# Anttwo/MACARONS

Measured on AMD Instinct MI355X. Metric: candidate-camera coverage-gain evals/sec (100k pts, 200 cams), higher is better.
Workload: dtype f32; 1 GPU; scorer: B=1 cloud x N=100000 points x C=200 cameras per GPU (BASELINE headline 100k pts / 200 cams), inputs resident in HBM; points=100000, cams_per_gpu=200, parallelism=camera-shard x1, streams=2

## Files before the change

### macarons_amd/csrc/networks.hip

```cpp
#include "nn_kernels.h"
#include "net_layout.h"
#include <cstdlib>
#include <algorithm>
#include <map>
#include <mutex>
#include <utility>

namespace mcr {

#ifdef MCR_DEV_LOCAL_PCT8
void launch_local_pct8(hipStream_t s, const float* offs, float* feat, int64_t ld_feat, int64_t S, const float* blob);
#define MCR_VARIANT8_OK(v) ((v) == 8)
#else
#define MCR_VARIANT8_OK(v) false
#endif
static int g_default_variant = []() {
    const char* e = getenv("MCR_LOCAL_PCT_VARIANT");
    const int v = e ? atoi(e) : 6;
    return (v == 1 || v == 5 || v == 6) ? v : 6;
}();
static thread_local int t_next_variant = 0;
static thread_local int t_variant = 0;
static thread_local int t_scope_depth = 0;
struct VariantScope {
// ... 474 lines not shown
        launch_linear3p(s, fP, W2, {fc2.b, ACT_GELU}, h128, T, 128, VIS_E, np);
        launch_linear3p(s, h128, W3, {fc3.b, ACT_NONE}, {out, 64}, T, 64, 128, np);
    } else {
        launch_layernorm(s, x, VIS_E, w.ng, w.nb, h, VIS_E, T, VIS_E);
        launch_linear(s, {h, VIS_E}, {fc1.w, VIS_E}, {fc1.b, ACT_GELU}, {ff, VIS_E}, T, 192, VIS_E, seq_route(N));
        launch_copy2d(s, view_harmonics, 64, ff + 192, VIS_E, T, 64);
        launch_linear(s, {ff, VIS_E}, {fc2.w, VIS_E}, {fc2.b, ACT_GELU}, {h, 128}, T, 128, VIS_E, seq_route(N));
        launch_linear(s, {h, 128}, {fc3.w, 128}, {fc3.b, ACT_NONE}, {out, 64}, T, 64, 128, N);
    }
    MCR_LAUNCH_CHECK("mcr_scone_vis_forward");
    return 0;
}

constexpr int OCC_CHUNK = 16384;
constexpr int FEAT = 1344;
constexpr size_t OCC_WS_SLACK = 8192 + 2 * 1024, OCC_RAGGED_WS_SLACK = 8192 + 1024;

struct OccHead {
    float *feat, *h1, *h2, *gfeat, *gbias;
    void* wplanes;
    HeadScratch planes() const { return HeadScratch{reinterpret_cast<_Float16*>(feat), reinterpret_cast<_Float16*>(h1), h2, wplanes}; }
};
static OccHead carve_occ_head(Arena& a, int64_t T, int64_t G) {
    OccHead w;
    w.feat = a.f(T * FEAT);
    w.h1 = a.f(T * 512);
    w.h2 = a.f(T * 256);
    w.gfeat = a.f(G * 512);
    w.gbias = a.f(G * 512);
    w.wplanes = a.bytes(linear3h_planes_bytes(512, 1344));
    return w;
}

struct OccSide { hipStream_t s = nullptr; hipEvent_t fork = nullptr, join = nullptr; };
static OccSide* occ_side(hipStream_t caller, int slot = 0) {
    static const bool on = []() { const char* e = getenv("MCR_OCC_OVERLAP"); return !(e && e[0] == '0'); }();
    if (!on) return nullptr;
    static std::mutex mu;
    static std::map<std::pair<std::pair<int, int>, hipStream_t>, OccSide> table;
    int dev = 0;
    if (hipGetDevice(&dev) != hipSuccess) return nullptr;
    std::lock_guard<std::mutex> lock(mu);
    OccSide& x = table[std::make_pair(std::make_pair(dev, slot), caller)];
    if (!x.s) {
        if (hipStreamCreateWithFlags(&x.s, hipStreamNonBlocking) != hipSuccess || hipEventCreateWithFlags(&x.fork, hipEventDisableTiming) != hipSuccess ||
            hipEventCreateWithFlags(&x.join, hipEventDisableTiming) != hipSuccess) {
            x.s = nullptr;
            return nullptr;
        }
    }
    return &x;
}
static hipStream_t fork_side(hipStream_t s, OccSide*& side) {
    if (side && hipEventRecord(side->fork, s) == hipSuccess && hipStreamWaitEvent(side->s, side->fork, 0) == hipSuccess) return side->s;
    side = nullptr;
    return s;
}
struct SideJoin {
    OccSide* side; hipStream_t s; bool recorded = false, joined = false;
    ~SideJoin() {
        if (!side || joined) return;
        if (!recorded) (void)hipEventRecord(side->join, side->s);
        (void)hipStreamWaitEvent(s, side->join, 0);
    }
};

static void run_global(hipStream_t gs, const OccW& w, const float* pc_global, int64_t G, int64_t Lg, const int* lens, const EncScratch& glob,
                       const OccHead& hd) {
    run_pct(gs, w.global, pc_global, hd.gfeat, 512, G, (int)Lg, 256, glob, lens);
    launch_linear(gs, {hd.gfeat, 512}, {w.lin1.w, 1856}, {nullptr, ACT_NONE}, {hd.gbias, 512}, G, 512, 512, 1);
}

static void head_linear(hipStream_t s, int which, Rows X, const LinW& lin, int64_t ldw, RowsOut Y, int64_t M, int N, int K, RowBias rb,
                        const void* const* head_planes, const float* head_inv_scales, void* wplanes) {
    const int variant = g_local_pct_variant;
    const int64_t ANY_M = (int64_t)1 << 40;
    const Rows W{lin.w, ldw};
    const Epilogue e{lin.b, ACT_GELU, {}, rb};
    if ((variant == 6 || variant == 7) && linear3h_applicable(X.p, X.ld, W.p, W.ld, ANY_M, N, K))
        launch_linear3h(s, X, head_weight_planes(s, which, lin, ldw, N, K, head_planes, head_inv_scales, wplanes), e, Y, M, N, K);
    else if (variant == 5 && linear3_applicable(X.p, X.ld, W.p, W.ld, ANY_M, N, K))
        launch_linear3(s, X, W, e, Y, M, N, K);
    else
        launch_linear(s, X, W, e, Y, M, N, K, 1);
}

static int run_occ_head(const char* who, hipStream_t s, const OccW& w, const float* x, const float* view_harmonics, int64_t T, const OccHead& hd,
                        int64_t rows_per_group, const int* row_group, const void* const* head_planes, const float* head_inv_scales, bool planes,
                        bool x_done, OccSide* side, SideJoin& side_join, int* range_flag, float* out) {
    bool join_failed = false;
    auto join = [&]() {
        if (side) {
            side_join.joined = true;
            join_failed = hipStreamWaitEvent(s, side->join, 0) != hipSuccess;
        }
    };
    if (planes)
        run_head_planes(s, x, view_harmonics, T, w.xe1, w.xe2, w.xe3, w.lin1, w.lin2, w.lin3, hd.gbias, rows_per_group, row_group, head_planes,
                        head_inv_scales, hd.planes(), out, join, x_done);
    else {
        launch_linear(s, {x, 3}, {w.xe1.w, 3}, {w.xe1.b, ACT_GELU}, {hd.h2, 128}, T, 128, 3, 1);
        head_linear(s, 0, {hd.h2, 128}, w.xe2, 128, {hd.h1, 256}, T, 256, 128, {}, head_planes, head_inv_scales, hd.wplanes);
        head_linear(s, 1, {hd.h1, 256}, w.xe3, 256, {hd.feat + 768, FEAT}, T, 512, 256, {}, head_planes, head_inv_scales, hd.wplanes);
        launch_copy2d(s, view_harmonics, 64, hd.feat + 1280, FEAT, T, 64);
        join();
        MCR_REQUIRE(!join_failed, "%s: side stream (join)", who);
        head_linear(s, 2, {hd.feat, FEAT}, {w.lin1.w + 512, w.lin1.b}, 1856, {hd.h1, 512}, T, 512, FEAT, {hd.gbias, rows_per_group, row_group},
                    head_planes, head_inv_scales, hd.wplanes);
        head_linear(s, 3, {hd.h1, 512}, w.lin2, 512, {hd.h2, 256}, T, 256, 512, {}, head_planes, head_inv_scales, hd.wplanes);
        launch_linear(s, {hd.h2, 256}, {w.lin3.w, 256}, {w.lin3.b, ACT_GELU}, {out, 1}, T, 1, 256, 1);
    }
    MCR_REQUIRE(!join_failed, "%s: side stream (join)", who);
    if (range_flag) launch_nonfinite_flag(s, out, T, range_flag);
    MCR_LAUNCH_CHECK(who);
    return 0;
}

struct OccLocal { float* offs; EncScratch pct; };
static OccLocal carve_occ_local(Arena& a, int64_t rows, bool layer_by_layer) {
    OccLocal w{};
    w.offs = a.f(rows * 16 * 3);
    if (layer_by_layer) w.pct = carve_enc(a, rows * 16, PCT_E);
    return w;
}
struct OccScratch {
    OccHead head;
    char *knn_q, *knn_c, *knn_park;
    size_t knn_c_bytes;
    EncScratch glob;
    Arena scratch;
};
static OccScratch carve_occ(Arena& a, int64_t B, int64_t Q, int64_t Lg) {
    OccScratch w;
    w.head = carve_occ_head(a, B * Q, B);
    w.knn_c_bytes = knn_grid_cloud_bytes(B, 16384);
    w.knn_q = (char*)a.bytes(knn_grid_query_bytes(B, Q));
    w.knn_c = (char*)a.bytes(3 * w.knn_c_bytes);
    w.knn_park = (char*)a.bytes(knn_grid_park_bytes());
    w.glob = carve_enc(a, B * Lg, PCT_E);
    w.scratch = a.rest();
    return w;
}
size_t mcr_scone_occ_workspace_bytes(int64_t B, int64_t Q, int64_t Lg) {
    const size_t local = std::max({measure(carve_occ_local, B * Q, false), measure(carve_occ_local, Q, false),
                                   measure(carve_occ_local, std::min<int64_t>(Q, OCC_CHUNK), true)});
    return measure(carve_occ, B, Q, Lg) + local + OCC_WS_SLACK;
}

int mcr_knn_points(const float* X, const float* pc, int64_t* idx, float* dists, float* pts, int64_t B, int64_t Q, int64_t M,
                   int k, int subtract_query, void* stream);

int mcr_scone_occ_forward_phase(const float* pc_global, int64_t Lg, const float* const* pc_scale, const int64_t* M_scale,
                                const float* x, const float* view_harmonics, float* out, int64_t B, int64_t Q,
                                const float* const* weights, int n_weights, const float* const* local_blobs,
                                const void* const* head_planes, const float* head_inv_scales, int* range_flag, void* workspace,
                                size_t workspace_bytes, int phase, void* stream) {
    const char* who = "mcr_scone_occ_forward";
    VariantScope variant_scope_;
    MCR_REQUIRE(phase >= 0 && phase <= 2, "mcr_scone_occ_forward: phase must be 0, 1 or 2");
    const bool early = phase != 2, late = phase != 1;
    MCR_REQUIRE(pc_scale && M_scale && x && weights && (!late || (pc_global && view_harmonics && out)), "mcr_scone_occ_forward: null pointer");
    MCR_REQUIRE(!head_planes || head_inv_scales, "mcr_scone_occ_forward: head_planes need head_inv_scales");
    if (check_table(who, OCC_TABLE, weights, n_weights, n_weights)) return 1;
    MCR_REQUIRE(B > 0 && Q > 0 && Lg > 0 && B <= 65535, "mcr_scone_occ_forward: bad problem size");
    MCR_REQUIRE(workspace && workspace_bytes >= mcr_scone_occ_workspace_bytes(B, Q, Lg), "mcr_scone_occ_forward: workspace too small");
    for (int i = 0; i < 3; ++i)
        MCR_REQUIRE((pc_scale[i] || (!late && i > 0)) && M_scale[i] >= 16, "mcr_scone_occ_forward: scale %d has %ld points (< k = 16)", i,
                    (long)M_scale[i]);
    hipStream_t s = (hipStream_t)stream;
    const OccW w = read_occ_table(weights, n_weights);
    Arena arena{(char*)workspace, workspace_bytes};
    const OccScratch ws = carve_occ(arena, B, Q, Lg);
    MCR_REQUIRE(arena.ok(), "mcr_scone_occ_forward: workspace overflow (global)");
    const OccHead& hd = ws.head;
    float* feat = hd.feat;

    OccSide* side = late ? occ_side(s) : nullptr;
    const hipStream_t gs = fork_side(s, side);
    SideJoin side_join{side, s};
    const bool fused_all = local_blobs && local_blobs[0] && local_blobs[1] && local_blobs[2];
    const int64_t qc = fused_all ? Q : std::min<int64_t>(Q, OCC_CHUNK);
    const bool planes = fused_all && fp16_planes_variant();
    const int64_t Tall = B * Q;
    const Planes featP = planes_over(hd.feat, Tall, FEAT);
    OccSide* xside = planes ? occ_side(s, 1) : nullptr;
    struct XJoin {
        OccSide* side; hipStream_t s; bool armed;
        bool wait() { if (!armed) return true; armed = false; return hipStreamWaitEvent(s, side->join, 0) == hipSuccess; }
        ~XJoin() { (void)wait(); }
    } x_join{xside, s, false};
    if (xside && early) {
        MCR_REQUIRE(hipEventRecord(xside->fork, s) == hipSuccess && hipStreamWaitEvent(xside->s, xside->fork, 0) == hipSuccess,
                    "mcr_scone_occ_forward: side stream (x embedding fork)");
        run_x_embedding_planes(xside->s, x, nullptr, B * Q, w.xe1, w.xe2, w.xe3, head_planes, head_inv_scales, hd.planes());
        MCR_REQUIRE(hipEventRecord(xside->join, xside->s) == hipSuccess, "mcr_scone_occ_forward: side stream (x embedding record)");
        x_join.armed = true;
    }
    if (late) {
        run_global(gs, w, pc_global, B, Lg, nullptr, ws.glob, hd);
        if (xside)
            launch_split_to_planes(gs, {view_harmonics, 64}, featP.cols(1280).keep(matrix_planes()), B * Q, 64);
    }
    if (side) {
        MCR_REQUIRE(hipEventRecord(side->join, side->s) == hipSuccess, "mcr_scone_occ_forward: side stream (record)");
        side_join.recorded = true;
    }
    const int* knn_qperm = nullptr;
    KnnGridCloud knn_clouds[3]{};
    int knn_slot[3] = {-1, -1, -1};
    if (qc == Q) {
        const float* g_pc[3]; int64_t g_M[3]; void* g_ws[3];
        int n_grid = 0;
        for (int sc = 0; sc < 3; ++sc)
            if (knn_grid_applicable(M_scale[sc], 16)) {
                g_pc[n_grid] = pc_scale[sc]; g_M[n_grid] = M_scale[sc]; g_ws[n_grid] = ws.knn_c + n_grid * ws.knn_c_bytes;
                knn_slot[sc] = n_grid++;
            }
        if (n_grid) {
            if (phase == 0) {
                knn_qperm = knn_grid_order_queries(s, x, B, Q, ws.knn_q, ws.knn_park);
                knn_grid_build_clouds(s, n_grid, g_pc, g_M, B, g_ws, knn_clouds);
            } else {
                const int first = early ? 0 : (knn_slot[0] >= 0 ? 1 : 0), count = early ? (knn_slot[0] >= 0 ? 1 : 0) : n_grid - first;
                OccSide* bside = early && count > 0 ? occ_side(s) : nullptr;
                const hipStream_t bs = fork_side(s, bside);
                knn_grid_build_clouds(bs, count, g_pc + first, g_M + first, B, g_ws + first, knn_clouds + first);
                const bool recorded = !bside || hipEventRecord(bside->join, bside->s) == hipSuccess;
                knn_qperm = knn_grid_order_queries(s, x, B, Q, ws.knn_q, ws.knn_park, early);
                const bool joined = !bside || hipStreamWaitEvent(s, bside->join, 0) == hipSuccess;
                MCR_REQUIRE(recorded && joined, "mcr_scone_occ_forward: side stream (cloud build)");
            }
            MCR_LAUNCH_CHECK("knn grid preparation");
        }
    }
    for (int sc = 0; sc < 3; ++sc) {
        if (sc == 0 ? !early : !late) continue;
        const bool grid_knn = knn_slot[sc] >= 0;
        const KnnGridCloud knn_cloud = grid_knn ? knn_clouds[knn_slot[sc]] : KnnGridCloud{};
        const bool fused = planes || (local_blobs && local_blobs[sc]);
        if (B > 1 && qc == Q && fused) {
            Arena a = ws.scratch;
            float* offs = carve_occ_local(a, Tall, false).offs;
            MCR_REQUIRE(a.ok(), "mcr_scone_occ_forward: workspace overflow (kNN)");
            if (grid_knn) {
                launch_knn16_grid(s, x, pc_scale[sc], M_scale[sc], knn_qperm, knn_cloud, 0, B, Q, nullptr, nullptr, offs, true, ws.knn_park, sc);
                MCR_LAUNCH_CHECK("knn_grid_kernel");
            } else if (int e = mcr_knn_points(x, pc_scale[sc], nullptr, nullptr, offs, B, Q, M_scale[sc], 16, 1, stream))
                return e;
            if (planes) run_local_pct(s, offs, nullptr, FEAT, Tall, local_blobs[sc], featP.cols(sc * 256));
            else run_local_pct(s, offs, feat + sc * 256, FEAT, Tall, local_blobs[sc]);
            continue;
        }
        for (int64_t q0 = 0; q0 < Q; q0 += qc) {
            const int64_t nq = std::min<int64_t>(qc, Q - q0);
            for (int64_t b = 0; b < B; ++b) {
                Arena a = ws.scratch;
                const OccLocal loc = carve_occ_local(a, nq, !fused);
                MCR_REQUIRE(a.ok(), fused ? "mcr_scone_occ_forward: workspace overflow (kNN)" : "mcr_scone_occ_forward: workspace overflow (local)");
                float* offs = loc.offs;
                if (grid_knn) {
                    launch_knn16_grid(s, x, pc_scale[sc], M_scale[sc], knn_qperm, knn_cloud, b, 1, Q, nullptr, nullptr, offs, true, ws.knn_park,
                                      (int)(sc * B + b));
                    MCR_LAUNCH_CHECK("knn_grid_kernel");
                } else if (int e = mcr_knn_points(x + (b * Q + q0) * 3, pc_scale[sc] + b * M_scale[sc] * 3, nullptr, nullptr, offs, 1, nq,
                                                  M_scale[sc], 16, 1, stream))
                    return e;
                if (planes)
                    run_local_pct(s, offs, nullptr, FEAT, nq, local_blobs[sc], featP.cols((b * Q + q0) * FEAT + sc * 256));
                else if (fused)
                    run_local_pct(s, offs, feat + (b * Q + q0) * FEAT + sc * 256, FEAT, nq, local_blobs[sc]);
                else
                    run_pct(s, w.local[sc], offs, feat + (b * Q + q0) * FEAT + sc * 256, FEAT, nq, 16, 128, loc.pct);
            }
        }
    }
    MCR_REQUIRE(x_join.wait(), "mcr_scone_occ_forward: side stream (x embedding join)");
    if (!late) {
        MCR_LAUNCH_CHECK("mcr_scone_occ_forward (phase 1)");
        return 0;
    }
    return run_occ_head(who, s, w, x, view_harmonics, Tall, hd, Q, nullptr, head_planes, head_inv_scales, planes, xside != nullptr, side,
                        side_join, range_flag, out);
}

int mcr_scone_occ_forward(const float* pc_global, int64_t Lg, const float* const* pc_scale, const int64_t* M_scale,
                          const float* x, const float* view_harmonics, float* out, int64_t B, int64_t Q,
                          const float* const* weights, int n_weights, const float* const* local_blobs,
                          const void* const* head_planes, const float* head_inv_scales, int* range_flag, void* workspace,
                          size_t workspace_bytes, void* stream) {
    return mcr_scone_occ_forward_phase(pc_global, Lg, pc_scale, M_scale, x, view_harmonics, out, B, Q, weights, n_weights, local_blobs,
                                       head_planes, head_inv_scales, range_flag, workspace, workspace_bytes, 0, stream);
}

struct OccRaggedScratch { OccHead head; EncScratch glob; float *offs, *knn_split; };
static OccRaggedScratch carve_occ_ragged(Arena& a, int64_t J, int64_t T, int64_t Lg) {
    OccRaggedScratch w;
    w.head = carve_occ_head(a, T, J);
    w.glob = carve_enc(a, J * Lg, PCT_E);
    w.offs = a.f(T * 16 * 3);
    w.knn_split = a.f(knn16_segmented_split_floats(T));
    return w;
}
size_t mcr_scone_occ_ragged_workspace_bytes(int64_t J, int64_t T, int64_t Lg) { return measure(carve_occ_ragged, J, T, Lg) + OCC_RAGGED_WS_SLACK; }
int mcr_knn_rows_per_block(void) { return knn_rows_per_block(); }

int mcr_scone_occ_forward_ragged_phase(const float* pc_global, const int* global_len, int64_t Lg, const float* const* pc_scale,
                                       const int64_t* const* scale_off, const float* x, const float* view_harmonics, const int* row_job,
                                       const int* knn_blocks, int64_t n_blocks, float* out, int64_t J, int64_t T,
                                       const float* const* weights, int n_weights, const float* const* local_blobs,
                                       const void* const* head_planes, const float* head_inv_scales, int* range_flag, void* workspace,
                                       size_t workspace_bytes, int phase, void* stream) {
// ... 61 lines not shown
```

### macarons_amd/nbv.py

```python

import torch

from . import dist as mdist
from .utility import scone_utils as su


class ViewStateGrid:

    def __init__(self, device, degree=8, n_elev=7, n_azim=14):
        self.n_elev, self.n_azim = n_elev, n_azim
        self.base_harmonics, self.h_polar, self.h_azim = su.get_all_harmonics_under_degree(degree, n_elev, n_azim, device)


_side_streams = {}


def _harmonics_beside(scone_occ, pc, Xl, harmonics_of):
    dev = Xl.device
    main = torch.cuda.current_stream(dev)
    fork = torch.cuda.Event()
    fork.record(main)
    begun = scone_occ.forward_begin(pc, Xl)
    if begun is None:
        return begun, harmonics_of(Xl)
    side = _side_streams.get((dev.index, main.cuda_stream))
    if side is None:
        side = _side_streams[(dev.index, main.cuda_stream)] = torch.cuda.Stream(device=dev)
    side.wait_event(fork)
    with torch.cuda.stream(side):
        vh = harmonics_of(Xl)
    main.wait_stream(side)
    vh.record_stream(main)
    return begun, vh


def _guarded(impl, scone_occ, range_guard, group, draws, device, scone_vis=None):
    from . import ops
    capturing = torch.cuda.is_current_stream_capturing()
    prev = scone_occ.range_guard
    guard = range_guard and prev != "off" and ops.current_variant() in (6, 7)
    scone_occ.range_guard = "defer" if (guard or prev != "off") else "off"
    vis_prev = None
    if scone_vis is not None and hasattr(scone_vis, "range_guard"):
        vis_prev = (scone_vis.range_guard, scone_vis._range_flag)
        scone_vis.range_guard = scone_occ.range_guard
    try:
        flagged = scone_occ.range_guard != "off" and ops.current_variant() in (6, 7)
        scone_occ.clear_range_flag(device if flagged else None)
        if vis_prev is not None:
            scone_vis._range_flag = scone_occ.range_flag()
        kw = draws() if (guard and not capturing) else {}
        out = impl(**kw)
        flag = scone_occ.range_flag() if ops.current_variant() in (6, 7) else None
        out["range_flag"] = flag
        if guard and not capturing:
# ... 56 lines not shown
    world, rank = mdist.group_world_rank(group)
    sharded = mdist.exchange_on(group)
    gather_rows, gather_best = mdist.allgather_rows, mdist.allgather_best
    if _emulate is not None:
        rank, world = _emulate
        sharded = True
        gather_rows = lambda t, n, g_=None: t.repeat(-(-n // max(t.shape[0], 1)), 1)[:n].contiguous()
        def gather_best(g_, c0_, grp=None):
            b_ = torch.max(g_, dim=1)
            return b_.values, b_.indices + c0_
    dev = X.device
    if view_proj is not None:
        X = su.filter_proxy_points(view_proj, X[0], pc.reshape(-1, 3), filter_tol=filter_tol)[0][None]
    Q = X.shape[1]
    if Q == 0:
        raise ValueError("nbv_step: no proxy point left to score (the proxy filter removed every point)")
    with torch.no_grad():
        q0, q1 = mdist.shard_range(Q, rank, world)
        Xl = X[:, q0:q1].contiguous()
        if sharded and _emulate is None and (occ_perms is None or samples is None):
            draw_perms, draw_u = occ_perms is None, samples is None
            if draw_perms:
                occ_perms = [p.to(dev) for p in scone_occ.draw_perms(pc.shape[1])]
            if draw_u:
                samples = torch.rand(seq_len, 1, device=dev)
            got_p, got_u = mdist.broadcast_draws(occ_perms if draw_perms else [], samples if draw_u else None, 0, group)
            if draw_perms:
                occ_perms = got_p
            if draw_u:
                samples = got_u
        if q1 > q0:
            harmonics_of = lambda pts: su.compute_view_harmonics(su.compute_view_state(pts, X_view, grid.n_elev, grid.n_azim),
                                                                 grid.base_harmonics, grid.h_polar, grid.h_azim, grid.n_elev, grid.n_azim)
            begun, vh_l = _harmonics_beside(scone_occ, pc, Xl, harmonics_of) if occ_perms is not None else (None, harmonics_of(Xl))
            if occ_perms is not None:
                occ_l = scone_occ(pc, Xl, vh_l, perms=occ_perms, begun=begun).view(-1, 1)
            else:
                occ_l = su.compute_occupancy_probability(scone_occ, pc, Xl, vh_l, max_points_per_pass=max_points_per_pass).view(-1, 1)
        else:
            vh_l = torch.zeros(1, 0, grid.base_harmonics.shape[0], dtype=torch.float32, device=dev)
            occ_l = torch.zeros(0, 1, dtype=torch.float32, device=dev)
        if sharded:
            occ = gather_rows(occ_l, Q, group)
            vh = None
        else:
            occ, vh = occ_l, vh_l[0]
        if samples is None:
            samples = torch.rand(seq_len, 1, device=dev)
        if vh is not None:
            proxy_points, vh_s, sample_idx, n_unique = su.sample_proxy_points(X[0], occ, vh, n_sample=seq_len, min_occ=min_occ,
                                                                              samples=samples, padded=True)
        else:
            from . import ops
            proxy_points, _, sample_idx, _, n_unique = ops.sample_proxy(X[0].contiguous(), occ.reshape(-1), None, samples.reshape(-1),
                                                                        min_occ, padded=True)
            vs_s = su.compute_view_state(proxy_points[None, :, :3].contiguous(), X_view, grid.n_elev, grid.n_azim)
            vh_s = su.compute_view_harmonics(vs_s, grid.base_harmonics, grid.h_polar, grid.h_azim, grid.n_elev, grid.n_azim)[0]
        sampled = (proxy_points, sample_idx)
        harm = scone_vis(proxy_points[None], view_harmonics=vh_s[None], lengths=n_unique)
        if true_monte_carlo_sampling:
            proxy_points, harm = proxy_points[sample_idx][None].contiguous(), harm[0][sample_idx][None].contiguous()
        else:
            k = int(n_unique)
            proxy_points, harm = proxy_points[:k][None].contiguous(), harm[:, :k].contiguous()
        C = X_cam.shape[0]
        c0, c1 = mdist.shard_range(C, rank, world)
        if c1 > c0:
# ... 46 lines not shown

def _nbv_step_batch(scone_occ, scone_vis, pc, X, X_view, X_cam, grid, seq_len=2048, min_occ=0.1, true_monte_carlo_sampling=True,
                    occ_perms=None, samples=None, group=None, return_samples=False):
    from . import ops
    world, rank = mdist.group_world_rank(group)
    dev = X.device
    B, Q, M, C = X.shape[0], X.shape[1], pc.shape[1], X_cam.shape[-2]
    if pc.shape[0] != B:
        raise ValueError("nbv_step_batch: pc and X must hold the same number of clouds")
    xch = mdist.exchange_on(group)
    by_cloud = xch and B >= world
    with torch.no_grad():
        if occ_perms is None or samples is None:
            dp, du = draw_batch(scone_occ, B, M, seq_len, dev)
            if xch:
                got_p, got_u = mdist.broadcast_draws(dp if occ_perms is None else [], du if samples is None else None, 0, group)
                dp, du = (got_p if occ_perms is None else dp), (got_u if samples is None else du)
            occ_perms = dp if occ_perms is None else occ_perms
            samples = du if samples is None else samples
        samples = samples.reshape(B, seq_len).to(dev)
        occ_perms = [p.to(dev) for p in occ_perms]
        b0, b1 = mdist.shard_range(B, rank, world) if by_cloud else (0, B)
        q0, q1 = (0, Q) if (by_cloud or not xch) else mdist.shard_range(Q, rank, world)
        c0, c1 = (0, C) if (by_cloud or not xch) else mdist.shard_range(C, rank, world)
        Bl = b1 - b0
        pc_l, X_b = pc[b0:b1].contiguous(), X[b0:b1].contiguous()
        Xv_l = X_view[b0:b1].contiguous() if X_view.dim() == 3 else X_view
        perms_l = [p[b0:b1] if p.dim() == 2 else p for p in occ_perms]
        u_l = samples[b0:b1].contiguous()
        vs_of = lambda pts: su.compute_view_harmonics(su.compute_view_state(pts, Xv_l, grid.n_elev, grid.n_azim), grid.base_harmonics,
                                                      grid.h_polar, grid.h_azim, grid.n_elev, grid.n_azim)
        if q1 > q0:
            Xl = X_b[:, q0:q1].contiguous()
            begun, vh_l = _harmonics_beside(scone_occ, pc_l, Xl, vs_of)
            occ_l = scone_occ(pc_l, Xl, vh_l, perms=perms_l, begun=begun).view(Bl, q1 - q0)
        else:
            vh_l, occ_l = None, torch.zeros(Bl, 0, dtype=torch.float32, device=dev)
        if q1 - q0 < Q:
            occ = mdist.allgather_rows(occ_l.t().contiguous(), Q, group).t().contiguous()
            vh_l = None
        else:
            occ = occ_l
        res, resh, inv, uniq, nu, _ = ops.sample_proxy_batched(X_b, occ, vh_l, u_l, min_occ)
        if resh is None:
            resh = vs_of(res[..., :3].contiguous())
        harm = scone_vis(res, view_harmonics=resh, lengths=nu)
        if true_monte_carlo_sampling:
            pts_s = torch.gather(res, 1, inv[..., None].expand(-1, -1, 4))
            harm_s = torch.gather(harm, 1, inv[..., None].expand(-1, -1, 64))
        else:
            raise NotImplementedError("nbv_step_batch scores the Monte-Carlo multiset (true_monte_carlo_sampling=True)")
        cams = X_cam[b0:b1] if X_cam.dim() == 3 else X_cam[None].expand(Bl, -1, -1)
        cams = cams[:, c0:c1].contiguous()
        gains = scone_vis.compute_coverage_gain(pts_s, harm_s, cams) if c1 > c0 else torch.zeros(Bl, 0, dtype=torch.float32, device=dev)
        record = None
        if not xch:
            flag = scone_occ.range_flag() if scone_occ.range_guard != "off" else None
            max_gain, nbv_idx, record = ops.nbv_decide(gains, nu.view(-1), flag)
        else:
            gains = torch.where(nu.view(-1, 1) < 1, torch.full_like(gains, float("nan")), gains)
            if by_cloud:
                rec = mdist.allgather_rows(ops.best_record(gains, 0), B, group)
                max_gain, nbv_idx = rec[:, 0].contiguous(), rec[:, 1].to(torch.int64)
                nbv_idx = torch.where(torch.isnan(max_gain), torch.full_like(nbv_idx, -1), nbv_idx)
            else:
                max_gain, nbv_idx = mdist.allgather_best(gains, c0, group)
                nbv_idx = torch.where(nu < 1, torch.full_like(nbv_idx, -1), nbv_idx)
# ... 55 lines not shown
```

### macarons_amd/networks/SconeOcc.py

```python
import numpy as np
import os
import torch
import torch.nn.functional as F
from torch import nn

from .. import autograd as A
from .. import ops, _lib
from .Attention import (Embedding, Encoder, FeedForward, MultiHeadSelfAttention, attention, knn_gather,
                        _f32c, _inference_only)
from ..utility.utils import get_knn_points
from .packing import encoder_weight_planes, padded_weight_planes, weight_planes, RangeGuard, BlobCache, HeadPlaneCache, TableCache, param_key, invalidate as _invalidate_key, freeze as _freeze_key


class XEmbedding(nn.Module):

    def __init__(self, x_dim, x_embedding_dim, dropout=None, gelu=True):
        super().__init__()
        if not gelu or dropout is not None:
            raise NotImplementedError("HIP path implements the GELU / no-dropout configuration")
        self.linear1 = nn.Linear(x_dim, x_embedding_dim // 4)
        self.linear2 = nn.Linear(x_embedding_dim // 4, x_embedding_dim // 2)
        self.linear3 = nn.Linear(x_embedding_dim // 2, x_embedding_dim)
        self.non_linear1, self.non_linear2, self.non_linear3 = nn.GELU(), nn.GELU(), nn.GELU()
        self.dropout = None
# ... 348 lines not shown
            return A.SconeOccRaggedFunction.apply(
                lambda: run(variant, None, ops.scone_occ_epoch(dev, h["arena"]) != h["epoch1"], None), self.weight_table, slots,
                [[s_[i] for s_ in sz] for i in range(self.n_scale)], h["query_sizes"], pc_global, g_len_d, [pc, pc1, pc2], d_row_job,
                x, view_harmonics, *params)
        flag = None
        guard = self._effective_guard()
        if variant in (6, 7) and guard != "off":
            if self._range_flag is None or self._range_flag.device != dev:
                self._range_flag = torch.zeros(1, dtype=torch.int32, device=dev)
            elif guard in ("sync", "async"):
                self._range_flag.zero_()
            flag = self._range_flag
        with torch.no_grad():
            res = run(variant, flag, ops.scone_occ_epoch(dev, h["arena"]) != h["epoch1"], out)
            if flag is not None and guard == "sync" and int(flag):
                with ops.variant(5):
                    res = run(5, None, True, out)
            elif flag is not None and guard == "async":
                self._post_range_check(flag)
        return res

    def scale_sizes(self, full_seq_len):
        ds, sizes = self.ds_factor(full_seq_len), [full_seq_len]
        for _ in range(self.n_scale - 1):
            sizes.append(sizes[-1] // ds)
        return sizes

    def _images(self, variant):
        key = param_key(self, self._key_cache)
        blobs = [c.get(t, variant, key) for c, t in zip(self._blob_caches, self.local_transformers)] if self.fused_local else None
        head = self._head_cache.get(self, key) if variant in (6, 7) else None
        return self._table_cache.get(self, self.weight_table_with_planes, key), blobs, head

    def forward_begin(self, pc, x):
        if not self._is_default_arch() or not self.fused_local or A.needs_grad(self, pc, x):
            return None
        variant = ops.current_variant()
        pc0, x_ = pc.contiguous(), x.contiguous()
        sizes = self.scale_sizes(pc.shape[1])
        if min(sizes) < self.k_for_knn:
            return None
        with torch.no_grad():
            table, blobs, head = self._images(variant)
            ops.scone_occ_forward(None, [pc0, None, None], x_, None, table, blobs, head, None, phase=1, M_scale=sizes, Lg=self.seq_len)
        return {"pc": pc0, "x": x_, "variant": variant, "sizes": sizes, "src": (pc, x), "epoch": ops.scone_occ_epoch(pc0.device, "scone_occ")}

    def forward(self, pc, x, view_harmonics, mask=None, verbose=False, perms=None, begun=None):
        if mask is not None:
            raise NotImplementedError("SconeOcc.forward(mask=...): upstream applies the same mask to sequences of 2048 and of 16 tokens")
        if not self._is_default_arch():
            raise NotImplementedError("the fused MI355X SconeOcc forward implements the reference's default architecture")
        n_clouds, full_seq_len = pc.shape[0], pc.shape[1]
        n_sample = x.shape[1]
        if perms is None:
            perms = self.draw_perms(full_seq_len)
        dev = pc.device
        L = _lib.lib()
        if self._effective_guard() == "async" and (self._range_pending or self._full_range):
            self.check_range()
        if self._full_range and ops.current_variant() in (6, 7):
            with ops.variant(5):
                return self.forward(pc, x, view_harmonics, mask, verbose, perms, None)
        variant = ops.current_variant()
        sizes = self.scale_sizes(full_seq_len)
        if begun is not None and not (begun["src"][0] is pc and begun["src"][1] is x and begun["variant"] == variant
                                      and begun["sizes"] == sizes and [p_.shape[-1] for p_ in perms] == [self.seq_len] + sizes[1:]
                                      and begun["epoch"] == ops.scone_occ_epoch(dev, "scone_occ")):
            begun = None
        pc_global = self._take(pc, perms[0])
        scales = [begun["pc"] if begun is not None else pc.contiguous()]
        for p in perms[1:]:
            scales.append(self._take(scales[-1], p))
        phase = 0
        if begun is not None:
            phase, x = 2, begun["x"]

        def run(variant, pc_global, scales, x_, vh_, flag, phase=0):
            table, blobs, head = self._images(variant)
            return ops.scone_occ_forward(pc_global, scales, x_, vh_, table, blobs, head, flag, phase=phase)

        flag = None
        guard = self._effective_guard()
        if variant in (6, 7) and guard != "off":
            if self._range_flag is None or self._range_flag.device != dev:
                self._range_flag = torch.zeros(1, dtype=torch.int32, device=dev)
            elif guard in ("sync", "async"):
                self._range_flag.zero_()
            flag = self._range_flag
        if A.needs_grad(self, pc, x, view_harmonics) and A.scone_occ_backward_mode() == "hip" and not pc.requires_grad:
            params, slots = self._grad_slots()
            res = A.SconeOccFunction.apply(lambda g_, sc_, x_, vh_: run(variant, g_, sc_, x_, vh_, None), self.weight_table, slots,
                                           self.k_for_knn, pc_global, scales, x, view_harmonics, *params)
        elif A.needs_grad(self, pc, x, view_harmonics):
            pidx = [p.to(dev) for p in perms]

            def clouds(pc_):
                sc = [pc_.contiguous()]
                for p in pidx[1:]:
                    sc.append(self._take(sc[-1], p))
                return self._take(pc_, pidx[0]), sc

            def hip(pc_, x_, vh_):
                g, sc = clouds(pc_)
                return run(variant, g, sc, x_, vh_, None)

            def composite(pc_, x_, vh_):
                g, sc = clouds(pc_)
                with torch.no_grad():
# ... 12 lines not shown
```

### macarons_amd/ops.py

```python
import os
import ctypes
import torch
import numpy as np

from ._lib import lib, check, MacaronsHipError, c_i64, c_int, c_size, c_vp, c_f32
from .utility.host import limit_host_threads

limit_host_threads()


def _stream():
    return c_vp(torch.cuda.current_stream().cuda_stream)


def _req(t, name, dtype=torch.float32):
    if not isinstance(t, torch.Tensor):
        raise TypeError(f"{name} must be a torch.Tensor")
    if not t.is_cuda:
        raise MacaronsHipError(f"{name} must live on a HIP device (got {t.device}); "
                               "the MI355X hot path has no CPU fallback")
    if t.dtype != dtype:
        raise TypeError(f"{name} must be {dtype} (got {t.dtype})")
    return t.contiguous()

# ... 610 lines not shown
        raise ValueError("colmax_backward: x, d_bcast and d_x must all be [S,L,E] (d_x contiguous float32)")
    if lens is not None:
        lens = _req(lens, "lens", torch.int32).reshape(-1)
        if lens.numel() != S:
            raise ValueError(f"lens must hold one length per sequence ({S}), got {lens.numel()}")
    with torch.cuda.device(x.device):
        check(lib().mcr_colmax_backward(_p(x), c_i64(E), _p(d_bcast), c_i64(E), _p(d_x), c_i64(E), c_i64(S), c_i64(L), c_int(E),
                                        _p(lens) if lens is not None else c_vp(0), _stream()), "mcr_colmax_backward")
    return d_x


def nonfinite_flag_(x, flag):
    x = _req(x, "x")
    if x.numel():
        with torch.cuda.device(x.device):
            check(lib().mcr_nonfinite_flag(_p(x), c_i64(x.numel()), _p(_req(flag, "flag", torch.int32)), _stream()), "mcr_nonfinite_flag")
    return flag


def local_pct_forward(offsets, blob):
    offsets, blob = _req(offsets, "offsets"), _req(blob, "blob")
    S = offsets.shape[0]
    if tuple(offsets.shape[1:]) != (16, 3):
        raise ValueError("offsets must be [S,16,3]")
    out = torch.empty((S, 256), dtype=torch.float32, device=offsets.device)
    with torch.cuda.device(offsets.device):
        check(_net(lib()).mcr_local_pct_forward(_p(offsets), _p(out), c_i64(256), c_i64(S), _p(blob), _stream()),
              "mcr_local_pct_forward")
    return out


def scone_occ_forward(pc_global, pc_scales, x, view_harmonics, weights, local_blobs=None, head_planes=None, range_flag=None, phase=0,
                      M_scale=None, Lg=None, out=None):
    late = phase != 1
    x = _req(x, "x")
    B, Q = x.shape[0], x.shape[1]
    if late:
        pc_global, view_harmonics = _req(pc_global, "pc_global"), _req(view_harmonics, "view_harmonics")
        pc_scales = [_req(p, "pc_scale") for p in pc_scales]
        Lg = pc_global.shape[1]
        M_scale = [p.shape[1] for p in pc_scales]
        if pc_global.shape[0] != B or len(pc_scales) != 3 or x.shape != (B, Q, 3) or view_harmonics.shape != (B, Q, 64):
            raise ValueError("SconeOcc HIP path needs 3 scales, x [B,Q,3] and view_harmonics [B,Q,64]")
    else:
        pc_scales = [_req(pc_scales[0], "pc_scale"), None, None]
        if x.shape != (B, Q, 3) or M_scale is None or len(M_scale) != 3 or Lg is None or pc_scales[0].shape[1] != M_scale[0]:
            raise ValueError("SconeOcc phase 1 needs x [B,Q,3], the whole cloud, the three scale sizes and Lg")
    L_ = lib()
    if late and out is None:
        out = torch.empty((B, Q, 1), dtype=torch.float32, device=x.device)
    nb = L_.mcr_scone_occ_workspace_bytes(c_i64(B), c_i64(Q), c_i64(Lg))
    ws = _workspace(x.device, nb, "scone_occ")
    _bump_epoch(x.device, "scone_occ")
    tab = _ptr_table(weights)
    sc_ptrs = (ctypes.c_void_p * 3)(*[p.data_ptr() if p is not None else None for p in pc_scales])
    sc_m = (ctypes.c_int64 * 3)(*[int(m) for m in M_scale])
    blobs = (ctypes.c_void_p * 3)(*[_req(b, "local_blob").data_ptr() for b in local_blobs]) if local_blobs else None
    with torch.cuda.device(x.device):
        check(_net(L_).mcr_scone_occ_forward_phase(_p(pc_global) if late else c_vp(0), c_i64(Lg), sc_ptrs, sc_m, _p(x),
                                             _p(view_harmonics) if late else c_vp(0), _p(out) if late else c_vp(0), c_i64(B),
                                             c_i64(Q), tab, c_int(_n_weights(weights)), blobs,
                                             head_planes[1] if head_planes is not None else None,
                                             head_planes[2] if head_planes is not None else None,
                                             _p(_req(range_flag, "range_flag", torch.int32)) if range_flag is not None else c_vp(0),
                                             _p(ws), c_size(ws.numel()), c_int(int(phase)), _stream()),
              "mcr_scone_occ_forward")
    return out


def scone_occ_forward_ragged(pc_global, global_len, pc_scales, scale_offsets, x, view_harmonics, row_job, knn_blocks, weights,
                             local_blobs, head_planes=None, range_flag=None, phase=0, Lg=None, out=None, arena="scone_occ_ragged"):
    x, view_harmonics = _req(x, "x"), _req(view_harmonics, "view_harmonics")
    row_job = _req(row_job, "row_job", torch.int32)
    knn_blocks = _req(knn_blocks, "knn_blocks", torch.int32)
    late = phase != 1
    pc_scales = [_req(p, "pc_scale") for p in (pc_scales if late else [pc_scales[0]] * 3)]
    scale_offsets = [_req(o, "scale_offsets", torch.int64) for o in (scale_offsets if late else [scale_offsets[0]] * 3)]
    J = scale_offsets[0].numel() - 1
    if late:
        pc_global, global_len = _req(pc_global, "pc_global"), _req(global_len, "global_len", torch.int32)
        Lg = pc_global.shape[1]
        if pc_global.shape[0] != J or global_len.numel() != J:
            raise ValueError("scone_occ_forward_ragged: pc_global [J,Lg,3], global_len [J]")
    T = x.shape[0]
    if x.shape != (T, 3) or view_harmonics.shape != (T, 64) or row_job.numel() != T:
        raise ValueError("scone_occ_forward_ragged: x [T,3], view_harmonics [T,64], row_job [T]")
    if any(o.numel() != J + 1 for o in scale_offsets) or knn_blocks.dim() != 2 or knn_blocks.shape[1] != 4:
        raise ValueError("scone_occ_forward_ragged: scale_offsets must be [J+1], knn_blocks [n_blocks,4]")
    L_ = lib()
    if late and out is None:
        out = torch.empty((T, 1), dtype=torch.float32, device=x.device)
    ws = _workspace(x.device, L_.mcr_scone_occ_ragged_workspace_bytes(c_i64(J), c_i64(T), c_i64(Lg)), arena)
# ... 914 lines not shown
```

Before: 5.154 million evals/s.

## Run scale-1/2 KNN searches and global transformer early on side streams

Adds phases 3 and 4 to the SconeOcc forward. When the permutations are known in forward_begin, the KNN searches for scales 1 and 2 run on a dedicated side stream into new workspace buffers, and the global transformer runs on another side stream, both overlapping the view-harmonics computation. The later phase reuses those results and only runs the local PCT encoders and head. This costs extra workspace, adds event bookkeeping across calls and checks that the perms tensors are unchanged.

```diff
diff --git a/macarons_amd/csrc/networks.hip b/macarons_amd/csrc/networks.hip
--- a/macarons_amd/csrc/networks.hip
+++ b/macarons_amd/csrc/networks.hip
@@ -530,7 +530,10 @@
     return w;
 }
 
-struct OccSide { hipStream_t s = nullptr; hipEvent_t fork = nullptr, join = nullptr; };
+struct OccSide {
+    hipStream_t s = nullptr; hipEvent_t fork = nullptr, join = nullptr;
+    hipEvent_t done[2] = {nullptr, nullptr}; bool pending = false, recorded = false;
+};
 static OccSide* occ_side(hipStream_t caller, int slot = 0) {
     static const bool on = []() { const char* e = getenv("MCR_OCC_OVERLAP"); return !(e && e[0] == '0'); }();
     if (!on) return nullptr;
@@ -542,7 +545,9 @@
     OccSide& x = table[std::make_pair(std::make_pair(dev, slot), caller)];
     if (!x.s) {
         if (hipStreamCreateWithFlags(&x.s, hipStreamNonBlocking) != hipSuccess || hipEventCreateWithFlags(&x.fork, hipEventDisableTiming) != hipSuccess ||
-            hipEventCreateWithFlags(&x.join, hipEventDisableTiming) != hipSuccess) {
+            hipEventCreateWithFlags(&x.join, hipEventDisableTiming) != hipSuccess ||
+            (slot == 2 && (hipEventCreateWithFlags(&x.done[0], hipEventDisableTiming) != hipSuccess ||
+                           hipEventCreateWithFlags(&x.done[1], hipEventDisableTiming) != hipSuccess))) {
             x.s = nullptr;
             return nullptr;
         }
@@ -561,6 +566,22 @@
         if (!recorded) (void)hipEventRecord(side->join, side->s);
         (void)hipStreamWaitEvent(s, side->join, 0);
     }
+};
+struct EarlyJoin {
+    OccSide *side, *global; hipStream_t s; bool keep = false;
+    bool join() {
+        bool ok = true;
+        if (side && side->pending) {
+            side->pending = false;
+            ok = (side->recorded || hipEventRecord(side->done[1], side->s) == hipSuccess) && hipStreamWaitEvent(s, side->done[1], 0) == hipSuccess;
+        }
+        if (global && global->pending) {
+            global->pending = false;
+            ok = hipEventRecord(global->join, global->s) == hipSuccess && hipStreamWaitEvent(s, global->join, 0) == hipSuccess && ok;
+        }
+        return ok;
+    }
+    ~EarlyJoin() { if (!keep) (void)join(); }
 };
 
 static void run_global(hipStream_t gs, const OccW& w, const float* pc_global, int64_t G, int64_t Lg, const int* lens, const EncScratch& glob,
@@ -623,8 +644,9 @@
 }
 struct OccScratch {
     OccHead head;
-    char *knn_q, *knn_c, *knn_park;
+    char *knn_q, *knn_c, *knn_park, *knn_park_early;
     size_t knn_c_bytes;
+    float* offs_early[2];
     EncScratch glob;
     Arena scratch;
 };
@@ -635,6 +657,8 @@
     w.knn_q = (char*)a.bytes(knn_grid_query_bytes(B, Q));
     w.knn_c = (char*)a.bytes(3 * w.knn_c_bytes);
     w.knn_park = (char*)a.bytes(knn_grid_park_bytes());
+    w.knn_park_early = (char*)a.bytes(knn_grid_park_bytes());
+    for (float*& o : w.offs_early) o = a.f(B * Q * 16 * 3);
     w.glob = carve_enc(a, B * Lg, PCT_E);
     w.scratch = a.rest();
     return w;
@@ -655,17 +679,26 @@
                                 size_t workspace_bytes, int phase, void* stream) {
     const char* who = "mcr_scone_occ_forward";
     VariantScope variant_scope_;
-    MCR_REQUIRE(phase >= 0 && phase <= 2, "mcr_scone_occ_forward: phase must be 0, 1 or 2");
-    const bool early = phase != 2, late = phase != 1;
-    MCR_REQUIRE(pc_scale && M_scale && x && weights && (!late || (pc_global && view_harmonics && out)), "mcr_scone_occ_forward: null pointer");
+    hipStream_t s = (hipStream_t)stream;
+    OccSide* eside = occ_side(s, 2);
+    EarlyJoin early_join{eside, occ_side(s), s};
+    if (phase != 4) MCR_REQUIRE(early_join.join(), "mcr_scone_occ_forward: side stream (stale early work)");
+    MCR_REQUIRE(phase >= 0 && phase <= 4, "mcr_scone_occ_forward: phase must be 0, 1, 2, 3 or 4");
+    MCR_REQUIRE(pc_scale && M_scale && x && weights, "mcr_scone_occ_forward: null pointer");
+    const bool fused_all = local_blobs && local_blobs[0] && local_blobs[1] && local_blobs[2];
+    if (!fused_all && phase >= 3) phase -= 2;
+    const bool early = phase != 2 && phase != 4, late = phase != 1 && phase != 3;
+    const bool search_early = fused_all && (phase == 0 || phase == 3), searched_early = phase == 4;
+    MCR_REQUIRE((pc_global || phase == 1) && (!late || (view_harmonics && out)), "mcr_scone_occ_forward: null pointer");
     MCR_REQUIRE(!head_planes || head_inv_scales, "mcr_scone_occ_forward: head_planes need head_inv_scales");
     if (check_table(who, OCC_TABLE, weights, n_weights, n_weights)) return 1;
     MCR_REQUIRE(B > 0 && Q > 0 && Lg > 0 && B <= 65535, "mcr_scone_occ_forward: bad problem size");
     MCR_REQUIRE(workspace && workspace_bytes >= mcr_scone_occ_workspace_bytes(B, Q, Lg), "mcr_scone_occ_forward: workspace too small");
     for (int i = 0; i < 3; ++i)
-        MCR_REQUIRE((pc_scale[i] || (!late && i > 0)) && M_scale[i] >= 16, "mcr_scone_occ_forward: scale %d has %ld points (< k = 16)", i,
+        MCR_REQUIRE((pc_scale[i] || (phase == 1 && i > 0)) && M_scale[i] >= 16, "mcr_scone_occ_forward: scale %d has %ld points (< k = 16)", i,
                     (long)M_scale[i]);
-    hipStream_t s = (hipStream_t)stream;
+    if (searched_early)
+        MCR_REQUIRE(!eside || eside->pending, "mcr_scone_occ_forward: phase 4 without the searches of a phase 3 on this stream");
     const OccW w = read_occ_table(weights, n_weights);
     Arena arena{(char*)workspace, workspace_bytes};
     const OccScratch ws = carve_occ(arena, B, Q, Lg);
@@ -676,7 +709,7 @@
     OccSide* side = late ? occ_side(s) : nullptr;
     const hipStream_t gs = fork_side(s, side);
     SideJoin side_join{side, s};
-    const bool fused_all = local_blobs && local_blobs[0] && local_blobs[1] && local_blobs[2];
+    if (side) side->pending = false;
     const int64_t qc = fused_all ? Q : std::min<int64_t>(Q, OCC_CHUNK);
     const bool planes = fused_all && fp16_planes_variant();
     const int64_t Tall = B * Q;
@@ -695,7 +728,7 @@
         x_join.armed = true;
     }
     if (late) {
-        run_global(gs, w, pc_global, B, Lg, nullptr, ws.glob, hd);
+        if (phase != 4) run_global(gs, w, pc_global, B, Lg, nullptr, ws.glob, hd);
         if (xside)
             launch_split_to_planes(gs, {view_harmonics, 64}, featP.cols(1280).keep(matrix_planes()), B * Q, 64);
     }
@@ -706,7 +739,7 @@
     const int* knn_qperm = nullptr;
     KnnGridCloud knn_clouds[3]{};
     int knn_slot[3] = {-1, -1, -1};
-    if (qc == Q) {
+    if (qc == Q && !searched_early) {
         const float* g_pc[3]; int64_t g_M[3]; void* g_ws[3];
         int n_grid = 0;
         for (int sc = 0; sc < 3; ++sc)
@@ -719,7 +752,8 @@
                 knn_qperm = knn_grid_order_queries(s, x, B, Q, ws.knn_q, ws.knn_park);
                 knn_grid_build_clouds(s, n_grid, g_pc, g_M, B, g_ws, knn_clouds);
             } else {
-                const int first = early ? 0 : (knn_slot[0] >= 0 ? 1 : 0), count = early ? (knn_slot[0] >= 0 ? 1 : 0) : n_grid - first;
+                const int first = early ? 0 : (knn_slot[0] >= 0 ? 1 : 0);
+                const int count = phase == 3 ? n_grid : early ? (knn_slot[0] >= 0 ? 1 : 0) : n_grid - first;
                 OccSide* bside = early && count > 0 ? occ_side(s) : nullptr;
                 const hipStream_t bs = fork_side(s, bside);
                 knn_grid_build_clouds(bs, count, g_pc + first, g_M + first, B, g_ws + first, knn_clouds + first);
@@ -731,8 +765,49 @@
             MCR_LAUNCH_CHECK("knn grid preparation");
         }
     }
-    for (int sc = 0; sc < 3; ++sc) {
-        if (sc == 0 ? !early : !late) continue;
+    hipStream_t es = s, gs3 = s;
+    if (search_early) {
+        OccSide* fs = eside;
+        es = fork_side(s, fs);
+        MCR_REQUIRE(fs == eside, "mcr_scone_occ_forward: side stream (early searches fork)");
+        if (eside) { eside->pending = true; eside->recorded = false; }
+    }
+    if (phase == 3) {
+        side_join.side = occ_side(s);
+        gs3 = fork_side(s, side_join.side);
+    }
+    auto run_side_work = [&]() -> int {
+        if (search_early) {
+            if (eside) (void)hipMemsetAsync(ws.knn_park_early, 0, 256, es);
+            char* park = eside ? ws.knn_park_early : ws.knn_park;
+            for (int sc = 1; sc < 3; ++sc) {
+                if (knn_slot[sc] >= 0) {
+                    launch_knn16_grid(es, x, pc_scale[sc], M_scale[sc], knn_qperm, knn_clouds[knn_slot[sc]], 0, B, Q, nullptr, nullptr,
+                                      ws.offs_early[sc - 1], true, park, sc);
+                    MCR_LAUNCH_CHECK("knn_grid_kernel");
+                } else if (int e = mcr_knn_points(x, pc_scale[sc], nullptr, nullptr, ws.offs_early[sc - 1], B, Q, M_scale[sc], 16, 1, es))
+                    return e;
+                if (eside)
+                    MCR_REQUIRE(hipEventRecord(eside->done[sc - 1], es) == hipSuccess, "mcr_scone_occ_forward: side stream (early searches record)");
+            }
+            if (eside) eside->recorded = true;
+        }
+        if (phase == 3) {
+            run_global(gs3, w, pc_global, B, Lg, nullptr, ws.glob, hd);
+            MCR_LAUNCH_CHECK("mcr_scone_occ_forward (global transformer)");
+        }
+        return 0;
+    };
+    auto run_scale = [&](int sc) -> int {
+        if (sc > 0 && (search_early || searched_early)) {
+            if (eside) {
+                MCR_REQUIRE(hipStreamWaitEvent(s, eside->done[sc - 1], 0) == hipSuccess, "mcr_scone_occ_forward: side stream (early searches join)");
+                if (sc == 2) eside->pending = false;
+            }
+            if (planes) run_local_pct(s, ws.offs_early[sc - 1], nullptr, FEAT, Tall, local_blobs[sc], featP.cols(sc * 256));
+            else run_local_pct(s, ws.offs_early[sc - 1], feat + sc * 256, FEAT, Tall, local_blobs[sc]);
+            return 0;
+        }
         const bool grid_knn = knn_slot[sc] >= 0;
         const KnnGridCloud knn_cloud = grid_knn ? knn_clouds[knn_slot[sc]] : KnnGridCloud{};
         const bool fused = planes || (local_blobs && local_blobs[sc]);
@@ -747,7 +822,7 @@
                 return e;
             if (planes) run_local_pct(s, offs, nullptr, FEAT, Tall, local_blobs[sc], featP.cols(sc * 256));
             else run_local_pct(s, offs, feat + sc * 256, FEAT, Tall, local_blobs[sc]);
-            continue;
+            return 0;
         }
         for (int64_t q0 = 0; q0 < Q; q0 += qc) {
             const int64_t nq = std::min<int64_t>(qc, Q - q0);
@@ -771,10 +846,19 @@
                     run_pct(s, w.local[sc], offs, feat + (b * Q + q0) * FEAT + sc * 256, FEAT, nq, 16, 128, loc.pct);
             }
         }
-    }
+        return 0;
+    };
+    if (early) {
+        if (int e = run_scale(0)) return e;
+        if (int e = run_side_work()) return e;
+    }
+    for (int sc = 1; late && sc < 3; ++sc)
+        if (int e = run_scale(sc)) return e;
     MCR_REQUIRE(x_join.wait(), "mcr_scone_occ_forward: side stream (x embedding join)");
     if (!late) {
         MCR_LAUNCH_CHECK("mcr_scone_occ_forward (phase 1)");
+        early_join.keep = true;
+        if (side_join.side) { side_join.side->pending = true; side_join.joined = true; }
         return 0;
     }
     return run_occ_head(who, s, w, x, view_harmonics, Tall, hd, Q, nullptr, head_planes, head_inv_scales, planes, xside != nullptr, side,
diff --git a/macarons_amd/nbv.py b/macarons_amd/nbv.py
--- a/macarons_amd/nbv.py
+++ b/macarons_amd/nbv.py
@@ -15,12 +15,12 @@
 _side_streams = {}
 
 
-def _harmonics_beside(scone_occ, pc, Xl, harmonics_of):
+def _harmonics_beside(scone_occ, pc, Xl, harmonics_of, perms=None):
     dev = Xl.device
     main = torch.cuda.current_stream(dev)
     fork = torch.cuda.Event()
     fork.record(main)
-    begun = scone_occ.forward_begin(pc, Xl)
+    begun = scone_occ.forward_begin(pc, Xl, perms)
     if begun is None:
         return begun, harmonics_of(Xl)
     side = _side_streams.get((dev.index, main.cuda_stream))
@@ -143,7 +143,7 @@
         if q1 > q0:
             harmonics_of = lambda pts: su.compute_view_harmonics(su.compute_view_state(pts, X_view, grid.n_elev, grid.n_azim),
                                                                  grid.base_harmonics, grid.h_polar, grid.h_azim, grid.n_elev, grid.n_azim)
-            begun, vh_l = _harmonics_beside(scone_occ, pc, Xl, harmonics_of) if occ_perms is not None else (None, harmonics_of(Xl))
+            begun, vh_l = _harmonics_beside(scone_occ, pc, Xl, harmonics_of, occ_perms) if occ_perms is not None else (None, harmonics_of(Xl))
             if occ_perms is not None:
                 occ_l = scone_occ(pc, Xl, vh_l, perms=occ_perms, begun=begun).view(-1, 1)
             else:
@@ -256,7 +256,7 @@
                                                       grid.h_polar, grid.h_azim, grid.n_elev, grid.n_azim)
         if q1 > q0:
             Xl = X_b[:, q0:q1].contiguous()
-            begun, vh_l = _harmonics_beside(scone_occ, pc_l, Xl, vs_of)
+            begun, vh_l = _harmonics_beside(scone_occ, pc_l, Xl, vs_of, perms_l)
             occ_l = scone_occ(pc_l, Xl, vh_l, perms=perms_l, begun=begun).view(Bl, q1 - q0)
         else:
             vh_l, occ_l = None, torch.zeros(Bl, 0, dtype=torch.float32, device=dev)
diff --git a/macarons_amd/networks/SconeOcc.py b/macarons_amd/networks/SconeOcc.py
--- a/macarons_amd/networks/SconeOcc.py
+++ b/macarons_amd/networks/SconeOcc.py
@@ -404,7 +404,12 @@
         head = self._head_cache.get(self, key) if variant in (6, 7) else None
         return self._table_cache.get(self, self.weight_table_with_planes, key), blobs, head
 
-    def forward_begin(self, pc, x):
+    @staticmethod
+    def _same_perms(searched, perms):
+        return searched is not None and len(searched) == len(perms) and all(
+            p is q and p._version == v for (q, v), p in zip(searched, perms))
+
+    def forward_begin(self, pc, x, perms=None):
         if not self._is_default_arch() or not self.fused_local or A.needs_grad(self, pc, x):
             return None
         variant = ops.current_variant()
@@ -412,10 +417,20 @@
         sizes = self.scale_sizes(pc.shape[1])
         if min(sizes) < self.k_for_knn:
             return None
+        scales, searched, pc_global = [pc0, None, None], None, None
+        if perms is not None and len(perms) == 3 and [p_.shape[-1] for p_ in perms[1:]] == sizes[1:]:
+            searched = [(p_, p_._version) for p_ in perms]
+            for i, p_ in enumerate(perms[1:], 1):
+                scales[i] = self._take(scales[i - 1], p_)
+            pc_global = self._take(pc, perms[0])
         with torch.no_grad():
             table, blobs, head = self._images(variant)
-            ops.scone_occ_forward(None, [pc0, None, None], x_, None, table, blobs, head, None, phase=1, M_scale=sizes, Lg=self.seq_len)
-        return {"pc": pc0, "x": x_, "variant": variant, "sizes": sizes, "src": (pc, x), "epoch": ops.scone_occ_epoch(pc0.device, "scone_occ")}
+            if searched is None:
+                ops.scone_occ_forward(None, scales, x_, None, table, blobs, head, None, phase=1, M_scale=sizes, Lg=self.seq_len)
+            else:
+                ops.scone_occ_forward(pc_global, scales, x_, None, table, blobs, head, None, phase=3, M_scale=sizes, Lg=pc_global.shape[1])
+        return {"pc": pc0, "x": x_, "variant": variant, "sizes": sizes, "src": (pc, x), "epoch": ops.scone_occ_epoch(pc0.device, "scone_occ"),
+                "searched": searched, "scales": scales, "pc_global": pc_global}
 
     def forward(self, pc, x, view_harmonics, mask=None, verbose=False, perms=None, begun=None):
         if mask is not None:
@@ -439,13 +454,17 @@
                                       and begun["sizes"] == sizes and [p_.shape[-1] for p_ in perms] == [self.seq_len] + sizes[1:]
                                       and begun["epoch"] == ops.scone_occ_epoch(dev, "scone_occ")):
             begun = None
-        pc_global = self._take(pc, perms[0])
-        scales = [begun["pc"] if begun is not None else pc.contiguous()]
-        for p in perms[1:]:
-            scales.append(self._take(scales[-1], p))
+        early = begun is not None and self._same_perms(begun["searched"], perms)
+        if early:
+            pc_global, scales = begun["pc_global"], list(begun["scales"])
+        else:
+            pc_global = self._take(pc, perms[0])
+            scales = [begun["pc"] if begun is not None else pc.contiguous()]
+            for p in perms[1:]:
+                scales.append(self._take(scales[-1], p))
         phase = 0
         if begun is not None:
-            phase, x = 2, begun["x"]
+            phase, x = (4 if early else 2), begun["x"]
 
         def run(variant, pc_global, scales, x_, vh_, flag, phase=0):
             table, blobs, head = self._images(variant)
diff --git a/macarons_amd/ops.py b/macarons_amd/ops.py
--- a/macarons_amd/ops.py
+++ b/macarons_amd/ops.py
@@ -666,7 +666,7 @@
 
 def scone_occ_forward(pc_global, pc_scales, x, view_harmonics, weights, local_blobs=None, head_planes=None, range_flag=None, phase=0,
                       M_scale=None, Lg=None, out=None):
-    late = phase != 1
+    late = phase not in (1, 3)
     x = _req(x, "x")
     B, Q = x.shape[0], x.shape[1]
     if late:
@@ -677,9 +677,13 @@
         if pc_global.shape[0] != B or len(pc_scales) != 3 or x.shape != (B, Q, 3) or view_harmonics.shape != (B, Q, 64):
             raise ValueError("SconeOcc HIP path needs 3 scales, x [B,Q,3] and view_harmonics [B,Q,64]")
     else:
-        pc_scales = [_req(pc_scales[0], "pc_scale"), None, None]
+        pc_scales = [_req(pc_scales[0], "pc_scale")] + ([_req(p, "pc_scale") for p in pc_scales[1:]] if phase == 3 else [None, None])
         if x.shape != (B, Q, 3) or M_scale is None or len(M_scale) != 3 or Lg is None or pc_scales[0].shape[1] != M_scale[0]:
             raise ValueError("SconeOcc phase 1 needs x [B,Q,3], the whole cloud, the three scale sizes and Lg")
+        if phase == 3:
+            pc_global = _req(pc_global, "pc_global")
+            if [p.shape[1] for p in pc_scales] != [int(m) for m in M_scale] or pc_global.shape[0] != B or pc_global.shape[1] != Lg:
+                raise ValueError("SconeOcc phase 3 needs pc_global [B,Lg,3] and the three clouds of the sizes in M_scale")
     L_ = lib()
     if late and out is None:
         out = torch.empty((B, Q, 1), dtype=torch.float32, device=x.device)
@@ -691,7 +695,7 @@
     sc_m = (ctypes.c_int64 * 3)(*[int(m) for m in M_scale])
     blobs = (ctypes.c_void_p * 3)(*[_req(b, "local_blob").data_ptr() for b in local_blobs]) if local_blobs else None
     with torch.cuda.device(x.device):
-        check(_net(L_).mcr_scone_occ_forward_phase(_p(pc_global) if late else c_vp(0), c_i64(Lg), sc_ptrs, sc_m, _p(x),
+        check(_net(L_).mcr_scone_occ_forward_phase(_p(pc_global) if late or phase == 3 else c_vp(0), c_i64(Lg), sc_ptrs, sc_m, _p(x),
                                              _p(view_harmonics) if late else c_vp(0), _p(out) if late else c_vp(0), c_i64(B),
                                              c_i64(Q), tab, c_int(_n_weights(weights)), blobs,
                                              head_planes[1] if head_planes is not None else None,
```

Result: no change. 5.166 million evals/s, median of 3 (+0.2%).
